# nju-websoft/OpenEA

Measured on AMD Instinct MI355X. Metric: training triples/sec (k=10 truncated negatives + limited loss + Adagrad), higher is better.
Workload: dtype f32; 1 GPU; BootEA/AlignE translational step, EN-FR-100K-V1 shape (synthetic), dim=100, GLOBAL batch=20000 positives (weak scaling: 20000 per GPU x 1 GPU), k=10, truncated eps=0.98; the same workload at every N (; global_batch=20000, entities=200000, parallelism=single

## Files before the change

openea_amd/csrc/sampler.hip:

```cpp
#include <stdlib.h>

#include <algorithm>

#include "common.h"

namespace {

__global__ void tripleset_clear(uint64_t *table, uint64_t capacity) {
    for (uint64_t i = (uint64_t)blockIdx.x * blockDim.x + threadIdx.x; i < capacity; i += (uint64_t)gridDim.x * blockDim.x)
        table[i] = OEA_EMPTY_KEY;
}

__global__ void tripleset_insert(const int32_t *__restrict__ triples, int64_t n, uint64_t *table, uint64_t capacity) {
    for (int64_t i = (int64_t)blockIdx.x * blockDim.x + threadIdx.x; i < n; i += (int64_t)gridDim.x * blockDim.x) {
        const uint64_t key = oea::pack_triple((uint32_t)triples[3 * i], (uint32_t)triples[3 * i + 1], (uint32_t)triples[3 * i + 2]);
        uint64_t s = oea::mix64(key) & (capacity - 1);
        for (;;) {
            const unsigned long long prev = atomicCAS((unsigned long long *)&table[s], (unsigned long long)OEA_EMPTY_KEY, (unsigned long long)key);
            if (prev == OEA_EMPTY_KEY || prev == key) break;
            s = (s + 1) & (capacity - 1);
        }
    }
}

__device__ __forceinline__ uint64_t filter_bit(uint64_t key, uint64_t bits) { return oea::mix64(key ^ 0x9E3779B97F4A7C15ull) & (bits - 1); }

__global__ void tripleset_filter_insert(const int32_t *__restrict__ triples, int64_t n, uint32_t *__restrict__ filter, uint64_t bits) {
    for (int64_t i = (int64_t)blockIdx.x * blockDim.x + threadIdx.x; i < n; i += (int64_t)gridDim.x * blockDim.x) {
        const uint64_t b = filter_bit(oea::pack_triple((uint32_t)triples[3 * i], (uint32_t)triples[3 * i + 1], (uint32_t)triples[3 * i + 2]), bits);
        atomicOr(&filter[b >> 5], 1u << (b & 31));
    }
}

__device__ __forceinline__ bool contains(const uint64_t *__restrict__ table, uint64_t capacity, const uint32_t *__restrict__ filter,
                                         uint64_t filter_bits, uint32_t h, uint32_t r, uint32_t t) {
    const uint64_t key = oea::pack_triple(h, r, t);
    if (filter) {
        const uint64_t b = filter_bit(key, filter_bits);
        if (!((filter[b >> 5] >> (b & 31)) & 1u)) return false;
    }
    uint64_t s = oea::mix64(key) & (capacity - 1);
    for (;;) {
        const uint64_t cur = table[s];
        if (cur == key) return true;
        if (cur == OEA_EMPTY_KEY) return false;
        s = (s + 1) & (capacity - 1);
    }
}

constexpr int kMaxK = 64;

template <int G>
__global__ __launch_bounds__(256) void sample_negatives_kernel(
    const int32_t *__restrict__ pos, int64_t n_pos, int64_t n_split, int k, oea_sampler_side side0,
    oea_sampler_side side1, uint32_t k0, uint32_t k1, uint32_t step, uint32_t pos_offset,
    int max_try, int32_t *__restrict__ out, int32_t *__restrict__ err_flag,
    const int64_t *__restrict__ seg_off, const int64_t *__restrict__ seg_split, int n_seg, const int32_t *__restrict__ replay) {
    const int lane = threadIdx.x % G;
    const uint32_t step_in = step;
    const int64_t n_split_in = n_split;
    for (int64_t p = ((int64_t)blockIdx.x * blockDim.x + threadIdx.x) / G; p < n_pos; p += (int64_t)gridDim.x * blockDim.x / G) {
    step = step_in;
    n_split = n_split_in;
    int64_t pl = p;
    if (seg_off) {
        const int64_t p0 = ((int64_t)(uint32_t)__builtin_amdgcn_readfirstlane((int)(p >> 32)) << 32) | (uint32_t)__builtin_amdgcn_readfirstlane((int)p);
        int lo = 0, hi = n_seg;
        while (hi - lo > 1) {
            const int mid = (lo + hi) >> 1;
            if (seg_off[mid] <= p0) lo = mid; else hi = mid;
        }
        int64_t first = seg_off[lo], split = seg_split[lo];
        int seg = lo;
        if (p >= seg_off[lo + 1]) {
            int l2 = lo;
            hi = n_seg;
            while (hi - l2 > 1) {
                const int mid = (l2 + hi) >> 1;
                if (seg_off[mid] <= p) l2 = mid; else hi = mid;
            }
            seg = l2; first = seg_off[l2]; split = seg_split[l2];
        }
        pl = p - first;
        n_split = split;
        step += (uint32_t)seg;
    }
    const oea_sampler_side &sd = pl < n_split ? side0 : side1;
    const uint64_t *__restrict__ table = sd.table;
    const uint64_t capacity = sd.capacity;
    const int32_t *__restrict__ entity_list = sd.entity_list;
    const int32_t *__restrict__ ent_pos = sd.ent_pos;
    const int32_t *__restrict__ nbr = sd.nbr;
    const uint32_t *__restrict__ filter = sd.filter;
    const uint64_t filter_bits = sd.filter_bits;
    const int n_ent_list = sd.n_ent_list, nbr_k = sd.nbr_k;
    const int32_t h = pos[3 * p], r = pos[3 * p + 1], t = pos[3 * p + 2];
    const bool h_has = nbr && ent_pos[h] >= 0, t_has = nbr && ent_pos[t] >= 0;
    const int32_t *hc = h_has ? nbr + (int64_t)ent_pos[h] * nbr_k : entity_list;
    const int32_t *tc = t_has ? nbr + (int64_t)ent_pos[t] * nbr_k : entity_list;
    const int hn = h_has ? nbr_k : n_ent_list, tn = t_has ? nbr_k : n_ent_list;
    const uint32_t c0 = (uint32_t)pl + pos_offset;
    const int gbase = (threadIdx.x & 63) / G * G;
    const unsigned long long gmask = (G == 64 ? ~0ull : ((1ull << G) - 1ull)) << gbase;
    int got = 0;
    for (int tr = 0; tr < max_try && got < k; ++tr) {
        const bool spare = k < G;
        uint4 w = oea::philox4x32_10(c0, step, (uint32_t)tr, (spare && lane != G - 1) ? 1u + (uint32_t)lane : 0u, k0, k1);
        const uint32_t side_word = spare ? (uint32_t)__shfl((int)w.x, (int)((threadIdx.x & 63) / G * G) + G - 1, 64) : w.x;
        const int32_t *rp = replay ? replay + ((int64_t)p * max_try + tr) * (1 + k) : nullptr;
        const bool corrupt_head = rp ? rp[0] != 0 : (side_word & 1u) != 0u;
        const int32_t *cand = corrupt_head ? hc : tc;
        const int nc = corrupt_head ? hn : tn;
        const int need = k - got;
        if (need > nc) { if (lane == 0) *err_flag = 1; break; }
        const bool active = lane < need;
        uint32_t att = 0;
        int32_t v = -1 - lane;
        if (active) {
            if (!spare) w = oea::philox4x32_10(c0, step, (uint32_t)tr, 1u + (uint32_t)lane, k0, k1);
            v = rp ? rp[1 + lane] : (int32_t)__umulhi(w.x, (uint32_t)nc);
            if (rp && (v < 0 || v >= nc)) { *err_flag = 2; v = 0; }
        }
        for (;;) {
            bool conflict = false;
            for (int q = 0; q < need; ++q) {
                const int32_t vq = __shfl(v, gbase + q, 64);
                conflict |= (q < lane) && (vq == v);
            }
            conflict &= active;
            if ((__ballot(conflict) & gmask) == 0ull) break;
            if (conflict) {
                ++att;
                w = oea::philox4x32_10(c0, step, (uint32_t)tr, 1u + (uint32_t)lane + 64u * att, k0, k1);
                v = (int32_t)__umulhi(w.x, (uint32_t)nc);
            }
        }
        bool accept = false;
        int32_t nh = h, nt = t;
        if (active) {
            const int32_t e = cand[v];
            nh = corrupt_head ? e : h;
            nt = corrupt_head ? t : e;
            accept = (tr == max_try - 1) || !contains(table, capacity, filter, filter_bits, (uint32_t)nh, (uint32_t)r, (uint32_t)nt);
        }
        const unsigned long long acc_mask = (__ballot(accept) & gmask) >> gbase;
        if (accept) {
            const int slot = got + __popcll(acc_mask & ((1ull << lane) - 1ull));
            struct __attribute__((packed, aligned(4))) Triple { int32_t h, r, t; };
            *reinterpret_cast<Triple *>(out + ((int64_t)p * k + slot) * 3) = Triple{nh, r, nt};
        }
        got += __popcll(acc_mask);
    }
    }
}

}

extern "C" {

uint64_t oea_tripleset_capacity(int64_t n) {
    uint64_t cap = 16;
    while (cap < 2ull * (uint64_t)(n > 1 ? n : 1)) cap *= 2;
    return cap;
}

int oea_tripleset_build(const int32_t *triples, int64_t n, uint64_t *table, uint64_t capacity, void *stream) {
    OEA_REQUIRE(table && (triples || n == 0), "null pointer");
    OEA_REQUIRE(capacity >= 2ull * (uint64_t)n && (capacity & (capacity - 1)) == 0, "capacity: power of two >= 2n");
    hipStream_t st = oea::as_stream(stream);
    tripleset_clear<<<1024, 256, 0, st>>>(table, capacity);
    if (n > 0) tripleset_insert<<<(unsigned)std::min<int64_t>(oea::ceil_div(n, 256), 4096), 256, 0, st>>>(triples, n, table, capacity);
    OEA_CHECK_HIP(hipGetLastError());
    return OEA_OK;
}

uint64_t oea_tripleset_filter_bits(uint64_t capacity) { return 8ull * capacity; }

int oea_tripleset_filter_build(const int32_t *triples, int64_t n, uint32_t *filter, uint64_t filter_bits, void *stream) {
    OEA_REQUIRE(filter && (triples || n == 0), "null pointer");
    OEA_REQUIRE(filter_bits >= 32 && (filter_bits & (filter_bits - 1)) == 0, "filter_bits: a power of two >= 32");
    hipStream_t st = oea::as_stream(stream);
    OEA_CHECK_HIP(hipMemsetAsync(filter, 0, (size_t)(filter_bits / 8), st));
    if (n > 0) tripleset_filter_insert<<<(unsigned)std::min<int64_t>(oea::ceil_div(n, 256), 4096), 256, 0, st>>>(triples, n, filter, filter_bits);
    OEA_CHECK_HIP(hipGetLastError());
    return OEA_OK;
}

int oea_sample_negatives(const int32_t *pos, int64_t n_pos, int32_t k, const uint64_t *table,
                         uint64_t capacity, const int32_t *entity_list, int32_t n_ent_list,
                         const int32_t *ent_pos, const int32_t *nbr, int32_t nbr_k, uint64_t seed,
                         uint32_t step, uint32_t pos_offset, int32_t max_try, int32_t *out,
                         int32_t *err_flag, void *stream) {
    oea_sampler_side sd{};
    sd.table = table; sd.capacity = capacity; sd.entity_list = entity_list; sd.ent_pos = ent_pos; sd.nbr = nbr;
    sd.n_ent_list = n_ent_list; sd.nbr_k = nbr_k;
    return oea_sample_negatives_pair(pos, n_pos, n_pos, k, &sd, &sd, seed, step, pos_offset, max_try, out, err_flag,
                                     stream);
}

static int check_side(const oea_sampler_side *s, int k) {
    OEA_REQUIRE(s && s->table && s->entity_list, "sampler side: null pointer");
    OEA_REQUIRE(s->nbr == nullptr || (s->ent_pos != nullptr && s->nbr_k > 0), "nbr needs ent_pos and nbr_k");
    OEA_REQUIRE((s->nbr ? s->nbr_k : s->n_ent_list) >= k && s->n_ent_list >= k, "Sample larger than population");
    return OEA_OK;
}

static int sample_impl(const int32_t *pos, int64_t n_pos, int64_t n_split, int32_t k,
                       const oea_sampler_side *side0, const oea_sampler_side *side1, uint64_t seed,
                       uint32_t step, uint32_t pos_offset, int32_t max_try, int32_t *out,
                       int32_t *err_flag, const int64_t *seg_off_dev, const int64_t *seg_split_dev, int n_seg,
                       void *stream, const int32_t *replay = nullptr) {
    OEA_REQUIRE(pos && out && err_flag, "null pointer");
    OEA_REQUIRE(k >= 1 && k <= kMaxK, "1 <= k <= 64");
    OEA_REQUIRE(max_try >= 1, "max_try >= 1");
    OEA_REQUIRE(n_split >= 0 && n_split <= n_pos, "0 <= n_split <= n_pos");
    int rc = check_side(side0, k);
    if (rc != OEA_OK) return rc;
    rc = check_side(side1, k);
    if (rc != OEA_OK) return rc;
    if (n_pos == 0) return OEA_OK;
    hipStream_t st = oea::as_stream(stream);
    static const int64_t cap_env = [] { const char *e = getenv("OEA_SAMPLER_CAP"); return e ? (int64_t)atoll(e) : (int64_t)0; }();
    const int64_t cap = (seg_off_dev && cap_env > 0) ? cap_env : ((int64_t)1 << 30);
    if (k <= 16)
        sample_negatives_kernel<16><<<(unsigned)std::min<int64_t>(oea::ceil_div(n_pos, 256 / 16), cap), 256, 0, st>>>(
            pos, n_pos, n_split, k, *side0, *side1, (uint32_t)seed, (uint32_t)(seed >> 32), step, pos_offset, max_try,
            out, err_flag, seg_off_dev, seg_split_dev, n_seg, replay);
    else
        sample_negatives_kernel<64><<<(unsigned)std::min<int64_t>(oea::ceil_div(n_pos, 256 / 64), cap), 256, 0, st>>>(
            pos, n_pos, n_split, k, *side0, *side1, (uint32_t)seed, (uint32_t)(seed >> 32), step, pos_offset, max_try,
            out, err_flag, seg_off_dev, seg_split_dev, n_seg, replay);
    OEA_CHECK_HIP(hipGetLastError());
    return OEA_OK;
}

int oea_sample_negatives_pair(const int32_t *pos, int64_t n_pos, int64_t n_split, int32_t k,
                              const oea_sampler_side *side0, const oea_sampler_side *side1, uint64_t seed,
                              uint32_t step, uint32_t pos_offset, int32_t max_try, int32_t *out,
                              int32_t *err_flag, void *stream) {
    return sample_impl(pos, n_pos, n_split, k, side0, side1, seed, step, pos_offset, max_try, out, err_flag, nullptr,
                       nullptr, 0, stream);
}

int oea_sample_negatives_replay(const int32_t *pos, int64_t n_pos, int32_t k, const uint64_t *table, uint64_t capacity,
                                const int32_t *entity_list, int32_t n_ent_list, const int32_t *ent_pos, const int32_t *nbr,
                                int32_t nbr_k, int32_t max_try, const int32_t *replay, int32_t *out, int32_t *err_flag, void *stream) {
    OEA_REQUIRE(replay, "replay record");
    oea_sampler_side sd{};
    sd.table = table; sd.capacity = capacity; sd.entity_list = entity_list; sd.ent_pos = ent_pos; sd.nbr = nbr;
    sd.n_ent_list = n_ent_list; sd.nbr_k = nbr_k;
    return sample_impl(pos, n_pos, n_pos, k, &sd, &sd, 0, 0u, 0u, max_try, out, err_flag, nullptr, nullptr, 0, stream, replay);
}

int oea_sample_negatives_epoch(const int32_t *pos_all, int64_t n_rows, const int64_t *offsets_dev,
                               const int64_t *splits_dev, int32_t steps, int32_t k, const oea_sampler_side *side0,
                               const oea_sampler_side *side1, uint64_t seed, uint32_t step_base, int32_t max_try,
                               int32_t *out_all, int32_t *err_flag, void *stream) {
    OEA_REQUIRE(offsets_dev && splits_dev && steps >= 1, "offsets / splits / steps");
    return sample_impl(pos_all, n_rows, 0, k, side0, side1, seed, step_base, 0u, max_try, out_all, err_flag, offsets_dev,
                       splits_dev, steps, stream);
}

}
```

Measured before the change: 290.4 million triples/s.

## Batch several positives per sampler group and use DPP for draw conflict checks

Adds an optional mode (OEA_SAMPLER_P) where each 16-lane group handles several positives, issuing their RNG, candidate gathers, filter probes and hash lookups together to overlap memory latency before falling back to per-round retries. For the 16-lane case the duplicate-draw check now uses DPP row shifts instead of a loop of wave shuffles. The batched path is off unless the environment variable is set, and it adds register pressure and code size.

```diff
diff --git a/openea_amd/csrc/sampler.hip b/openea_amd/csrc/sampler.hip
--- a/openea_amd/csrc/sampler.hip
+++ b/openea_amd/csrc/sampler.hip
@@ -32,6 +32,16 @@
     }
 }
 
+__device__ __forceinline__ bool table_holds(const uint64_t *__restrict__ table, uint64_t capacity, uint64_t key) {
+    uint64_t s = oea::mix64(key) & (capacity - 1);
+    for (;;) {
+        const uint64_t cur = table[s];
+        if (cur == key) return true;
+        if (cur == OEA_EMPTY_KEY) return false;
+        s = (s + 1) & (capacity - 1);
+    }
+}
+
 __device__ __forceinline__ bool contains(const uint64_t *__restrict__ table, uint64_t capacity, const uint32_t *__restrict__ filter,
                                          uint64_t filter_bits, uint32_t h, uint32_t r, uint32_t t) {
     const uint64_t key = oea::pack_triple(h, r, t);
@@ -39,117 +49,252 @@
         const uint64_t b = filter_bit(key, filter_bits);
         if (!((filter[b >> 5] >> (b & 31)) & 1u)) return false;
     }
-    uint64_t s = oea::mix64(key) & (capacity - 1);
+    return table_holds(table, capacity, key);
+}
+
+constexpr int kMaxK = 64;
+
+template <int S>
+__device__ __forceinline__ bool row_earlier_holds(int32_t v, int k) {
+    if constexpr (S >= 16) {
+        return false;
+    } else {
+        if (S >= k) return false;
+        const int32_t vq = __builtin_amdgcn_update_dpp((int)0x80000000, v, 0x110 + S, 0xf, 0xf, false);
+        return (vq == v) | row_earlier_holds<S + 1>(v, k);
+    }
+}
+
+template <int G>
+__device__ __forceinline__ bool earlier_holds(int32_t v, int k, int need, int lane, int gbase) {
+    if constexpr (G == 16) {
+        return row_earlier_holds<1>(v, k);
+    } else {
+        bool conflict = false;
+        for (int q = 0; q < need; ++q) {
+            const int32_t vq = __shfl(v, gbase + q, 64);
+            conflict |= (q < lane) && (vq == v);
+        }
+        return conflict;
+    }
+}
+
+template <int G>
+__device__ __forceinline__ int32_t settle_draws(int32_t v, bool active, int nc, int k, int need, int lane, int gbase, unsigned long long gmask,
+                                                uint32_t c0, uint32_t step, uint32_t tr, uint32_t k0, uint32_t k1) {
+    uint32_t att = 0;
     for (;;) {
-        const uint64_t cur = table[s];
-        if (cur == key) return true;
-        if (cur == OEA_EMPTY_KEY) return false;
-        s = (s + 1) & (capacity - 1);
-    }
-}
-
-constexpr int kMaxK = 64;
+        const bool conflict = earlier_holds<G>(v, k, need, lane, gbase) && active;
+        if ((__ballot(conflict) & gmask) == 0ull) break;
+        if (conflict) {
+            ++att;
+            const uint4 w = oea::philox4x32_10(c0, step, tr, 1u + (uint32_t)lane + 64u * att, k0, k1);
+            v = (int32_t)__umulhi(w.x, (uint32_t)nc);
+        }
+    }
+    return v;
+}
+
+struct __attribute__((packed, aligned(4))) Triple { int32_t h, r, t; };
+
+struct Row {
+    int32_t h, r, t, eh, et;
+    uint32_t c0, step;
+    bool s1;
+};
+
+__device__ __forceinline__ oea_sampler_side pick_side(bool second, const oea_sampler_side &a, const oea_sampler_side &b) {
+    oea_sampler_side s;
+    s.table = second ? b.table : a.table;
+    s.capacity = second ? b.capacity : a.capacity;
+    s.entity_list = second ? b.entity_list : a.entity_list;
+    s.ent_pos = second ? b.ent_pos : a.ent_pos;
+    s.nbr = second ? b.nbr : a.nbr;
+    s.n_ent_list = second ? b.n_ent_list : a.n_ent_list;
+    s.nbr_k = second ? b.nbr_k : a.nbr_k;
+    s.filter = second ? b.filter : a.filter;
+    s.filter_bits = second ? b.filter_bits : a.filter_bits;
+    return s;
+}
 
 template <int G>
+__device__ __forceinline__ bool sample_round(const oea_sampler_side &sd, const Row &rw, int64_t p, int k, uint32_t k0, uint32_t k1, int tr,
+                                             int max_try, int lane, int gbase, unsigned long long gmask,
+                                             const int32_t *__restrict__ replay, int32_t *__restrict__ out, int32_t *__restrict__ err_flag,
+                                             int &got) {
+    const bool spare = k < G;
+    uint4 w = oea::philox4x32_10(rw.c0, rw.step, (uint32_t)tr, (spare && lane != G - 1) ? 1u + (uint32_t)lane : 0u, k0, k1);
+    const uint32_t side_word = spare ? (uint32_t)__shfl((int)w.x, gbase + G - 1, 64) : w.x;
+    const int32_t *rp = replay ? replay + ((int64_t)p * max_try + tr) * (1 + k) : nullptr;
+    const bool corrupt_head = rp ? rp[0] != 0 : (side_word & 1u) != 0u;
+    const int32_t crow = corrupt_head ? rw.eh : rw.et;
+    const int32_t *cand = crow >= 0 ? sd.nbr + (int64_t)crow * sd.nbr_k : sd.entity_list;
+    const int nc = crow >= 0 ? sd.nbr_k : sd.n_ent_list;
+    const int need = k - got;
+    if (need > nc) { if (lane == 0) *err_flag = 1; return false; }
+    const bool active = lane < need;
+    int32_t v = -1 - lane;
+    if (active) {
+        if (!spare) w = oea::philox4x32_10(rw.c0, rw.step, (uint32_t)tr, 1u + (uint32_t)lane, k0, k1);
+        v = rp ? rp[1 + lane] : (int32_t)__umulhi(w.x, (uint32_t)nc);
+        if (rp && (v < 0 || v >= nc)) { *err_flag = 2; v = 0; }
+    }
+    v = settle_draws<G>(v, active, nc, k, need, lane, gbase, gmask, rw.c0, rw.step, (uint32_t)tr, k0, k1);
+    bool accept = false;
+    int32_t nh = rw.h, nt = rw.t;
+    if (active) {
+        const int32_t e = cand[v];
+        nh = corrupt_head ? e : rw.h;
+        nt = corrupt_head ? rw.t : e;
+        accept = (tr == max_try - 1) || !contains(sd.table, sd.capacity, sd.filter, sd.filter_bits, (uint32_t)nh, (uint32_t)rw.r, (uint32_t)nt);
+    }
+    const unsigned long long acc_mask = (__ballot(accept) & gmask) >> gbase;
+    if (accept) {
+        const int slot = got + __popcll(acc_mask & ((1ull << lane) - 1ull));
+        *reinterpret_cast<Triple *>(out + ((int64_t)p * k + slot) * 3) = Triple{nh, rw.r, nt};
+    }
+    got += __popcll(acc_mask);
+    return true;
+}
+
+template <int G, int P>
 __global__ __launch_bounds__(256) void sample_negatives_kernel(
     const int32_t *__restrict__ pos, int64_t n_pos, int64_t n_split, int k, oea_sampler_side side0,
     oea_sampler_side side1, uint32_t k0, uint32_t k1, uint32_t step, uint32_t pos_offset,
     int max_try, int32_t *__restrict__ out, int32_t *__restrict__ err_flag,
     const int64_t *__restrict__ seg_off, const int64_t *__restrict__ seg_split, int n_seg, const int32_t *__restrict__ replay) {
     const int lane = threadIdx.x % G;
-    const uint32_t step_in = step;
-    const int64_t n_split_in = n_split;
-    for (int64_t p = ((int64_t)blockIdx.x * blockDim.x + threadIdx.x) / G; p < n_pos; p += (int64_t)gridDim.x * blockDim.x / G) {
-    step = step_in;
-    n_split = n_split_in;
-    int64_t pl = p;
+    const int gbase = (threadIdx.x & 63) / G * G;
+    const unsigned long long gmask = (G == 64 ? ~0ull : ((1ull << G) - 1ull)) << gbase;
+    const int64_t n_groups = (n_pos + P - 1) / P;
+    for (int64_t g = ((int64_t)blockIdx.x * blockDim.x + threadIdx.x) / G; g < n_groups; g += (int64_t)gridDim.x * blockDim.x / G) {
+    const int64_t pg = g * P;
+    int seg0 = 0;
+    int64_t first0 = 0, split0 = n_split, next0 = 0;
     if (seg_off) {
-        const int64_t p0 = ((int64_t)(uint32_t)__builtin_amdgcn_readfirstlane((int)(p >> 32)) << 32) | (uint32_t)__builtin_amdgcn_readfirstlane((int)p);
+        const int64_t p0 = ((int64_t)(uint32_t)__builtin_amdgcn_readfirstlane((int)(pg >> 32)) << 32) | (uint32_t)__builtin_amdgcn_readfirstlane((int)pg);
         int lo = 0, hi = n_seg;
         while (hi - lo > 1) {
             const int mid = (lo + hi) >> 1;
             if (seg_off[mid] <= p0) lo = mid; else hi = mid;
         }
-        int64_t first = seg_off[lo], split = seg_split[lo];
-        int seg = lo;
-        if (p >= seg_off[lo + 1]) {
-            int l2 = lo;
-            hi = n_seg;
+        seg0 = lo; first0 = seg_off[lo]; split0 = seg_split[lo]; next0 = seg_off[lo + 1];
+    }
+    Row rw[P];
+    int got[P];
+    int64_t pj[P];
+#pragma unroll
+    for (int j = 0; j < P; ++j) {
+        const int64_t p = pg + j;
+        pj[j] = p;
+        got[j] = p < n_pos ? 0 : k;
+        int64_t first = first0, split = split0;
+        int seg = seg0;
+        if (seg_off && p < n_pos && p >= next0) {
+            int l2 = seg0, hi = n_seg;
             while (hi - l2 > 1) {
                 const int mid = (l2 + hi) >> 1;
                 if (seg_off[mid] <= p) l2 = mid; else hi = mid;
             }
             seg = l2; first = seg_off[l2]; split = seg_split[l2];
         }
-        pl = p - first;
-        n_split = split;
-        step += (uint32_t)seg;
-    }
-    const oea_sampler_side &sd = pl < n_split ? side0 : side1;
-    const uint64_t *__restrict__ table = sd.table;
-    const uint64_t capacity = sd.capacity;
-    const int32_t *__restrict__ entity_list = sd.entity_list;
-    const int32_t *__restrict__ ent_pos = sd.ent_pos;
-    const int32_t *__restrict__ nbr = sd.nbr;
-    const uint32_t *__restrict__ filter = sd.filter;
-    const uint64_t filter_bits = sd.filter_bits;
-    const int n_ent_list = sd.n_ent_list, nbr_k = sd.nbr_k;
-    const int32_t h = pos[3 * p], r = pos[3 * p + 1], t = pos[3 * p + 2];
-    const bool h_has = nbr && ent_pos[h] >= 0, t_has = nbr && ent_pos[t] >= 0;
-    const int32_t *hc = h_has ? nbr + (int64_t)ent_pos[h] * nbr_k : entity_list;
-    const int32_t *tc = t_has ? nbr + (int64_t)ent_pos[t] * nbr_k : entity_list;
-    const int hn = h_has ? nbr_k : n_ent_list, tn = t_has ? nbr_k : n_ent_list;
-    const uint32_t c0 = (uint32_t)pl + pos_offset;
-    const int gbase = (threadIdx.x & 63) / G * G;
-    const unsigned long long gmask = (G == 64 ? ~0ull : ((1ull << G) - 1ull)) << gbase;
-    int got = 0;
-    for (int tr = 0; tr < max_try && got < k; ++tr) {
-        const bool spare = k < G;
-        uint4 w = oea::philox4x32_10(c0, step, (uint32_t)tr, (spare && lane != G - 1) ? 1u + (uint32_t)lane : 0u, k0, k1);
-        const uint32_t side_word = spare ? (uint32_t)__shfl((int)w.x, (int)((threadIdx.x & 63) / G * G) + G - 1, 64) : w.x;
-        const int32_t *rp = replay ? replay + ((int64_t)p * max_try + tr) * (1 + k) : nullptr;
-        const bool corrupt_head = rp ? rp[0] != 0 : (side_word & 1u) != 0u;
-        const int32_t *cand = corrupt_head ? hc : tc;
-        const int nc = corrupt_head ? hn : tn;
-        const int need = k - got;
-        if (need > nc) { if (lane == 0) *err_flag = 1; break; }
-        const bool active = lane < need;
-        uint32_t att = 0;
-        int32_t v = -1 - lane;
-        if (active) {
-            if (!spare) w = oea::philox4x32_10(c0, step, (uint32_t)tr, 1u + (uint32_t)lane, k0, k1);
-            v = rp ? rp[1 + lane] : (int32_t)__umulhi(w.x, (uint32_t)nc);
-            if (rp && (v < 0 || v >= nc)) { *err_flag = 2; v = 0; }
-        }
-        for (;;) {
-            bool conflict = false;
-            for (int q = 0; q < need; ++q) {
-                const int32_t vq = __shfl(v, gbase + q, 64);
-                conflict |= (q < lane) && (vq == v);
+        const int64_t pl = p - first;
+        rw[j].s1 = !(pl < split);
+        rw[j].c0 = (uint32_t)pl + pos_offset;
+        rw[j].step = step + (uint32_t)seg;
+    }
+#pragma unroll
+    for (int j = 0; j < P; ++j) {
+        const bool on = got[j] < k;
+        rw[j].h = on ? pos[3 * pj[j]] : 0;
+        rw[j].r = on ? pos[3 * pj[j] + 1] : 0;
+        rw[j].t = on ? pos[3 * pj[j] + 2] : 0;
+    }
+    bool on0 = false, on1 = false;
+#pragma unroll
+    for (int j = 0; j < P; ++j) { on0 |= got[j] < k && !rw[j].s1; on1 |= got[j] < k && rw[j].s1; }
+    const bool wave1 = __ballot(on1) != 0ull, mixed = wave1 && __ballot(on0) != 0ull;
+    const oea_sampler_side su = pick_side(wave1, side0, side1);
+    if (P > 1 && !mixed) {
+#pragma unroll
+        for (int j = 0; j < P; ++j) {
+            const bool rows = got[j] < k && su.nbr != nullptr;
+            rw[j].eh = rows ? su.ent_pos[rw[j].h] : -1;
+            rw[j].et = rows ? su.ent_pos[rw[j].t] : -1;
+        }
+    } else {
+#pragma unroll
+        for (int j = 0; j < P; ++j) {
+            const oea_sampler_side sd = pick_side(rw[j].s1, side0, side1);
+            const bool rows = got[j] < k && sd.nbr != nullptr;
+            rw[j].eh = rows ? sd.ent_pos[rw[j].h] : -1;
+            rw[j].et = rows ? sd.ent_pos[rw[j].t] : -1;
+        }
+    }
+    if constexpr (P > 1) if (!mixed) {
+        const oea_sampler_side &sd = su;
+        static_assert(G == 16, "several positives per group: the 16-lane form only");
+        const bool spare = k < G, last = max_try == 1;
+        uint32_t wx[P];
+        int32_t v[P], e[P];
+        uint32_t fw[P];
+#pragma unroll
+        for (int j = 0; j < P; ++j)
+            wx[j] = oea::philox4x32_10(rw[j].c0, rw[j].step, 0u, (spare && lane != G - 1) ? 1u + (uint32_t)lane : 0u, k0, k1).x;
+        const int32_t *cand[P];
+        bool head[P], active[P];
+#pragma unroll
+        for (int j = 0; j < P; ++j) {
+            const uint32_t side_word = spare ? (uint32_t)__shfl((int)wx[j], gbase + G - 1, 64) : wx[j];
+            const int32_t *rp = replay ? replay + (int64_t)pj[j] * max_try * (1 + k) : nullptr;
+            const bool on = got[j] < k;
+            head[j] = (rp && on) ? rp[0] != 0 : (side_word & 1u) != 0u;
+            const int32_t crow = head[j] ? rw[j].eh : rw[j].et;
+            cand[j] = crow >= 0 ? sd.nbr + (int64_t)crow * sd.nbr_k : sd.entity_list;
+            const int nc = crow >= 0 ? sd.nbr_k : sd.n_ent_list;
+            active[j] = on && lane < k;
+            if (on && k > nc) {
+                if (lane == 0) *err_flag = 1;
+                got[j] = k;
+                active[j] = false;
             }
-            conflict &= active;
-            if ((__ballot(conflict) & gmask) == 0ull) break;
-            if (conflict) {
-                ++att;
-                w = oea::philox4x32_10(c0, step, (uint32_t)tr, 1u + (uint32_t)lane + 64u * att, k0, k1);
-                v = (int32_t)__umulhi(w.x, (uint32_t)nc);
+            v[j] = -1 - lane;
+            if (active[j]) {
+                if (!spare) wx[j] = oea::philox4x32_10(rw[j].c0, rw[j].step, 0u, 1u + (uint32_t)lane, k0, k1).x;
+                v[j] = rp ? rp[1 + lane] : (int32_t)__umulhi(wx[j], (uint32_t)nc);
+                if (rp && (v[j] < 0 || v[j] >= nc)) { *err_flag = 2; v[j] = 0; }
             }
-        }
-        bool accept = false;
-        int32_t nh = h, nt = t;
-        if (active) {
-            const int32_t e = cand[v];
-            nh = corrupt_head ? e : h;
-            nt = corrupt_head ? t : e;
-            accept = (tr == max_try - 1) || !contains(table, capacity, filter, filter_bits, (uint32_t)nh, (uint32_t)r, (uint32_t)nt);
-        }
-        const unsigned long long acc_mask = (__ballot(accept) & gmask) >> gbase;
-        if (accept) {
-            const int slot = got + __popcll(acc_mask & ((1ull << lane) - 1ull));
-            struct __attribute__((packed, aligned(4))) Triple { int32_t h, r, t; };
-            *reinterpret_cast<Triple *>(out + ((int64_t)p * k + slot) * 3) = Triple{nh, r, nt};
-        }
-        got += __popcll(acc_mask);
+            v[j] = settle_draws<G>(v[j], active[j], nc, k, k, lane, gbase, gmask, rw[j].c0, rw[j].step, 0u, k0, k1);
+        }
+#pragma unroll
+        for (int j = 0; j < P; ++j) e[j] = active[j] ? cand[j][v[j]] : 0;
+        uint64_t key[P];
+#pragma unroll
+        for (int j = 0; j < P; ++j) {
+            key[j] = oea::pack_triple((uint32_t)(head[j] ? e[j] : rw[j].h), (uint32_t)rw[j].r, (uint32_t)(head[j] ? rw[j].t : e[j]));
+            fw[j] = (active[j] && !last) ? ~0u : 0u;
+            if (fw[j] && sd.filter) {
+                const uint64_t b = filter_bit(key[j], sd.filter_bits);
+                fw[j] = (sd.filter[b >> 5] >> (b & 31)) & 1u;
+            }
+        }
+#pragma unroll
+        for (int j = 0; j < P; ++j) {
+            const bool accept = active[j] && !(fw[j] && table_holds(sd.table, sd.capacity, key[j]));
+            const unsigned long long acc_mask = (__ballot(accept) & gmask) >> gbase;
+            if (accept) {
+                const int slot = __popcll(acc_mask & ((1ull << lane) - 1ull));
+                *reinterpret_cast<Triple *>(out + ((int64_t)pj[j] * k + slot) * 3) =
+                    Triple{head[j] ? e[j] : rw[j].h, rw[j].r, head[j] ? rw[j].t : e[j]};
+            }
+            if (got[j] < k) got[j] = __popcll(acc_mask);
+        }
+    }
+#pragma unroll
+    for (int j = 0; j < P; ++j) {
+        const oea_sampler_side sd = pick_side(rw[j].s1, side0, side1);
+        for (int tr = (P > 1 && !mixed) ? 1 : 0; tr < max_try && got[j] < k; ++tr)
+            if (!sample_round<G>(sd, rw[j], pj[j], k, k0, k1, tr, max_try, lane, gbase, gmask, replay, out, err_flag, got[j])) break;
     }
     }
 }
@@ -222,14 +367,21 @@
     hipStream_t st = oea::as_stream(stream);
     static const int64_t cap_env = [] { const char *e = getenv("OEA_SAMPLER_CAP"); return e ? (int64_t)atoll(e) : (int64_t)0; }();
     const int64_t cap = (seg_off_dev && cap_env > 0) ? cap_env : ((int64_t)1 << 30);
-    if (k <= 16)
-        sample_negatives_kernel<16><<<(unsigned)std::min<int64_t>(oea::ceil_div(n_pos, 256 / 16), cap), 256, 0, st>>>(
+    const char *p_str = getenv("OEA_SAMPLER_P");
+    const int p_env = p_str ? atoi(p_str) : 0;
+    OEA_REQUIRE(p_env == 0 || p_env == 1 || p_env == 2 || p_env == 4 || p_env == 8, "OEA_SAMPLER_P: 1, 2, 4 or 8");
+    const int P = (k <= 16 && p_env) ? p_env : 1;
+    auto launch = [&](auto kernel, int G, int per) {
+        const int64_t groups = oea::ceil_div(n_pos, (int64_t)per);
+        kernel<<<(unsigned)std::min<int64_t>(oea::ceil_div(groups, (int64_t)(256 / G)), cap), 256, 0, st>>>(
             pos, n_pos, n_split, k, *side0, *side1, (uint32_t)seed, (uint32_t)(seed >> 32), step, pos_offset, max_try,
             out, err_flag, seg_off_dev, seg_split_dev, n_seg, replay);
-    else
-        sample_negatives_kernel<64><<<(unsigned)std::min<int64_t>(oea::ceil_div(n_pos, 256 / 64), cap), 256, 0, st>>>(
-            pos, n_pos, n_split, k, *side0, *side1, (uint32_t)seed, (uint32_t)(seed >> 32), step, pos_offset, max_try,
-            out, err_flag, seg_off_dev, seg_split_dev, n_seg, replay);
+    };
+    if (k > 16) launch(sample_negatives_kernel<64, 1>, 64, 1);
+    else if (P == 1) launch(sample_negatives_kernel<16, 1>, 16, 1);
+    else if (P == 2) launch(sample_negatives_kernel<16, 2>, 16, 2);
+    else if (P == 4) launch(sample_negatives_kernel<16, 4>, 16, 4);
+    else launch(sample_negatives_kernel<16, 8>, 16, 8);
     OEA_CHECK_HIP(hipGetLastError());
     return OEA_OK;
 }
```

After: 294.4 million triples/s (median of 6 runs). 1.4% higher.
